# Abolfazlmsl/Oriented-Object-Detection

Hardware: AMD Instinct MI355X
Metric: 416px tiles/sec (whole node), YOLOv11n-OBB 3ch (higher is better)
Workload: dtype f32; 1 GPU; YOLOv11n-OBB 3ch 416x416 tiled inference, single-scale (BASELINE configs[1]): forward + decode + ProbIoU NMS + border filter + per-tile merge + final polygon-IoU merge; step_pipelining=True, nc=12, weights=synthetic seeded, cls bias -8 (no checkpoint offline), final_detections=12170

## Files before the change

### oriented-object-detection_amd/csrc/ctx.h

```cpp
#pragma once
#include <hip/hip_runtime.h>

#include <cstdarg>
#include <cstdint>
#include <cstdio>
#include <map>
#include <memory>
#include <string>
#include <vector>

#include "../../include/obbhip.h"

namespace obb {
struct Model;
struct EngineOpts {
    bool tail = true, tail16 = true, bneck = true, bneck_cv2 = true, c3kimg = true, dwpw = true, upfold = true, stem = true, front = true, pair = true, hmerge = true,
         sppf_fuse = true, attn_mfma = true, xtile = true, nitile = true, nc2 = true, blk32 = true, c3k2f = true, pw32 = true, graph = true;
    int fwd_split = 0 , microbatch = 1024;
};
}

struct obb_ctx {
    int device = 0;
    std::string err;
    struct Slot { void *p = nullptr; size_t bytes = 0; };
    std::vector<Slot> ws;
    std::shared_ptr<obb::Model> model;
    std::map<int, std::shared_ptr<obb::Model>> slots;
    int slot = 0;
    bool opt_f16 = true;
    bool opt_f32 = false;
    obb::EngineOpts opt;
    void *workspace(int slot, size_t bytes);
    ~obb_ctx();
};

namespace obb {
int set_error(obb_ctx *ctx, int code, const char *fmt, ...);
extern thread_local std::string g_tls_error;

#define OBB_HIP(ctx, call)                                                                                  \
    do {                                                                                                    \
        hipError_t e_ = (call);                                                                             \
        if (e_ != hipSuccess)                                                                               \
            return obb::set_error(ctx, OBB_ERR_HIP, "%s failed: %s (%s:%d)", #call, hipGetErrorString(e_), \
                                  __FILE__, __LINE__);                                                      \
    } while (0)

#define OBB_REQUIRE(ctx, cond, ...)                                      \
    do {                                                                 \
        if (!(cond)) return obb::set_error(ctx, OBB_ERR_INVALID, __VA_ARGS__); \
    } while (0)

#define OBB_LAUNCH_CHECK(ctx) OBB_HIP(ctx, hipGetLastError())

enum { WS_GEOM_A = 0, WS_GEOM_B, WS_GEOM_C, WS_GEOM_D, WS_GEOM_E, WS_NMS_A, WS_NMS_B, WS_NMS_C, WS_NMS_D, WS_SURV_A, WS_SURV_B, WS_SEL, WS_DT, WS_TRAIN_A, WS_TRAIN_B, WS_TRAIN_C, WS_TRAIN_D, WS_TRAIN_E, WS_TRAIN_F, WS_COUNT };

inline int64_t cdiv(int64_t a, int64_t b) { return (a + b - 1) / b; }
}
```

### oriented-object-detection_amd/csrc/engine.hip

```cpp
#include <algorithm>
#include <cmath>
#include <cstdlib>
#include <cstring>
#include <map>
#include <memory>
#include <string>
#include <tuple>

#include "bneck.h"
#include "c3k2f32.h"
#include "c3kimg.h"
#include "ctx.h"
#include "dwpw.h"
#include "f32path.h"
#include "front.h"
#include "nnops.h"
#include "pw32.h"
#include "stem.h"

namespace obb {

static constexpr int kRegMax = 16;

struct ConvRecord {
    std::string name;
    int c1, c2, k, s, g, act;
    const float *w, *b;
};

struct Buf {
    int H, W, C;
    bool f32;
    bool virt = false;
    int va_buf = -1, va_co = 0, va_C = 0, vb_buf = -1, vb_co = 0, vb_C = 0;
    int blk = 0;
    int blk32 = 0;
    std::string name;
    int64_t off = 0;
    void *p = nullptr;
    int64_t per_img() const { return (int64_t)H * W * C; }
};

struct Slice { int buf = -1, co = 0, C = 0; };

enum OpType { OP_CONV32, OP_STEM32, OP_C3K2F32, OP_PW32, OP_CONV, OP_DW, OP_POOL, OP_UP, OP_ATTN, OP_STEM, OP_SPPF, OP_BNECK, OP_C3KIMG, OP_DWPW, OP_FRONT };

struct Op {
    OpType type;
    std::string name;
    Slice in, out, res;
    int H = 0, W = 0;
    int Ho = 0, Wo = 0;
    ConvLaunch conv;
    Conv32Launch c32;
    Stem32Launch stem32;
    Pw32Launch pw32;
    C3k2F32Launch c3k2f;
    StemLaunch stem;
    FrontLaunch front;
    BneckLaunch bneck;
    C3kImgLaunch c3kimg;
    DwPwLaunch dwpw;
    double macs = 0;
    bool one_d = false;
    bool vin = false;
    const bf16_t *dw_w = nullptr;
    const float *dw_b = nullptr;
    const float *dw_w32 = nullptr;
    int act = 0;
    int N = 0, nh = 0, kd = 0, hd = 0;
    int head_level = -1;
    bool emit_cmax = false;
    int lane = 0;
    int wait_feat = -1;
    int signal_feat = -1;
};

struct Plan {
    int h = 0, w = 0, A = 0, no = 0, no_pad = 0;
    std::vector<Buf> bufs;
    std::vector<Op> ops;
    std::map<std::string, Slice> named;
    std::vector<void *> dev_allocs;
    int lvl_off[3] = {0, 0, 0};
    int cmax_mask = 0;
    int cap = 0;
    void *slab = nullptr;
    int64_t bytes_per_img = 0;
    double macs_per_img = 0;
    static constexpr int kLanes = 4;
    hipStream_t lanes[kLanes] = {};
    hipEvent_t ev_feat[kLanes] = {}, ev_done[kLanes] = {};
    typedef std::tuple<int, const void *, void *, void *> GraphKey;
    std::map<GraphKey, hipGraphExec_t> graphs;
    std::map<GraphKey, int> seen;
    std::vector<GraphKey> graph_order;
    void drop_graphs() {
        for (auto &kv : graphs) (void)hipGraphExecDestroy(kv.second);
        graphs.clear();
        seen.clear();
        graph_order.clear();
    }
    ~Plan() {
        drop_graphs();
        for (int i = 0; i < kLanes; ++i) {
            if (lanes[i]) (void)hipStreamDestroy(lanes[i]);
            if (ev_feat[i]) (void)hipEventDestroy(ev_feat[i]);
            if (ev_done[i]) (void)hipEventDestroy(ev_done[i]);
        }
        for (void *p : dev_allocs) (void)hipFree(p);
        if (slab) (void)hipFree(slab);
    }
};

struct Model {
// ... 317 lines not shown
            op.name = name + "+" + tail_name;
            P.macs_per_img += (double)op.Ho * op.Wo * r2->c2 * r->c2;
            P.ops.push_back(op);
            if (act16) P.named[tail_name] = out;
            return;
        }
        P.ops.push_back(op);
        P.named[name] = out;
    }

    void dwconv(const std::string &name, Slice in, int H, int W, Slice out, Slice res = Slice()) {
        const ConvRecord *r = rec(name);
        if (!r || err) return;
        if (r->g != r->c1 || r->c1 != r->c2 || r->k != 3 || r->s != 1 || r->c1 != in.C || out.C != in.C) {
            err = set_error(ctx, OBB_ERR_FORMAT, "record %s: not a depthwise 3x3 matching the graph", name.c_str());
            return;
        }
        if (M.f32 && (P.bufs[in.buf].blk32 || P.bufs[out.buf].blk32)) { err = set_error(ctx, OBB_ERR_STATE, "depthwise layer %s on a channel-blocked buffer", name.c_str()); return; }
        int C = in.C;
        std::vector<bf16_t> w((size_t)9 * C + 8, 0);
        std::vector<float> b((size_t)C + 8, 0.f);
        for (int c = 0; c < C; ++c) {
            for (int t = 0; t < 9; ++t) w[(size_t)t * C + c] = host_to_half(r->w[(size_t)c * 9 + t], M.f16);
            b[c] = r->b[c];
        }
        Op op;
        op.type = OP_DW; op.name = name; op.in = in; op.out = out; op.res = res; op.H = H; op.W = W; op.Ho = H; op.Wo = W;
        op.act = r->act;
        if (M.f32) {
            std::vector<float> w32((size_t)9 * C + 8, 0.f);
            for (int c = 0; c < C; ++c)
                for (int t = 0; t < 9; ++t) w32[(size_t)t * C + c] = r->w[(size_t)c * 9 + t];
            op.dw_w32 = upload(w32);
        } else op.dw_w = upload(w);
        op.dw_b = upload(b);
        P.macs_per_img += (double)H * W * C * 9;
        P.ops.push_back(op);
        P.named[name] = out;
    }

    bool dwpw32(const std::string &dwname, const std::string &pwname, Slice in, int H, int W, Slice out, const char *tailname, int head_level) {
        const ConvRecord *rd = rec(dwname), *rp = rec(pwname), *rt = tailname ? rec(tailname) : nullptr;
        if (!(M.tail && M.o.dwpw) || !rd || !rp || (tailname && !rt) || err) return false;
        if (in.buf < 0 || P.bufs[in.buf].virt || rd->g != rd->c1 || rd->c1 != rd->c2 || rd->k != 3 || rd->s != 1 || rd->c1 != in.C || rp->g != 1 || rp->k != 1 || rp->s != 1 ||
            rp->c1 != in.C)
            return false;
        if (rt && (rt->g != 1 || rt->k != 1 || rt->s != 1 || rt->act || rt->c1 != rp->c2 || head_level < 0)) return false;
        if (!rt && (out.buf < 0 || P.bufs[out.buf].virt || out.C != rp->c2)) return false;
        const Conv32Tiling t = plan_dwpw32(in.C, rp->c2, H, W);
        if (t.TH == 0 || (rt && !conv32_tail_supported(t, rp->c2, rt->c2)) || (rt && rt->c2 > 16)) return false;
        Op op;
        op.type = OP_CONV32; op.name = dwname + "+" + pwname + (rt ? std::string("+") + tailname : std::string()); op.in = in; op.out = out;
        op.H = H; op.W = W; op.Ho = H; op.Wo = W; op.head_level = rt ? head_level : -1; op.one_d = false;
        Conv32Launch &L = op.c32;
        L.ks = 1; L.stride = 1; L.cin = in.C; L.cout = rp->c2; L.act = rp->act; L.dw = 1; L.dw_act = rd->act;
        L.TH = t.TH; L.TW = t.TW; L.CK = t.CK; L.WC = t.WC; L.MFM = t.MFM; L.NI = 1;
        L.Hin = L.Hout = H; L.Win = L.Wout = W;
        L.tiles_y = (H + t.TH - 1) / t.TH; L.tiles_x = 1;
        L.wpk = upload(pack_dwpw32_weights(rp->w, rp->c2, in.C, rd->w, rd->b, t));
        std::vector<float> bias32(((size_t)rp->c2 + 63) / 64 * 64 + 64, 0.f);
        for (int c = 0; c < rp->c2; ++c) bias32[c] = rp->b[c];
        L.bias = upload(bias32);
        op.macs = (double)H * W * (9.0 * in.C + (double)in.C * rp->c2);
        if (rt) {
            const Conv32Tiling t2{1, 1, rp->c2, 1, 1, 1};
            L.tail_w = upload(pack_conv32_weights(rt->w, rt->c2, rp->c2, 1, t2, nullptr, false));
            std::vector<float> b2(((size_t)rt->c2 + 63) / 64 * 64 + 64, 0.f);
            for (int c = 0; c < rt->c2; ++c) b2[c] = rt->b[c];
            L.tail_b = upload(b2);
            L.tail_cout = rt->c2; L.tail_act = 0;
            if (out.buf == -2 && out.co == 4 * kRegMax) { op.emit_cmax = true; P.cmax_mask |= 1 << head_level; }
            op.macs += (double)H * W * rt->c1 * rt->c2;
        }
        P.macs_per_img += op.macs;
        P.ops.push_back(op);
        if (!rt) P.named[pwname] = out;
        return true;
    }

    bool dwpw(const std::string &dwname, const std::string &pwname, Slice in, int H, int W, Slice out, const char *tailname = nullptr, int head_level = -1) {
        if (M.f32) return dwpw32(dwname, pwname, in, H, W, out, tailname, head_level);
        const bool on = M.tail && M.o.dwpw;
        const ConvRecord *rd = rec(dwname), *rp = rec(pwname), *rt = tailname ? rec(tailname) : nullptr;
        if (!on || !rd || !rp || (tailname && !rt) || err) return false;
        if (in.buf < 0 || P.bufs[in.buf].blk || P.bufs[in.buf].virt || rd->g != rd->c1 || rd->c1 != rd->c2 || rd->k != 3 || rd->s != 1 || rd->c1 != in.C || !rd->act ||
            rp->g != 1 || rp->k != 1 || rp->s != 1 || !rp->act || rp->c1 != in.C)
            return false;
        if (rt && (rt->g != 1 || rt->k != 1 || rt->s != 1 || rt->act || rt->c1 != rp->c2 || head_level < 0)) return false;
        if (!rt && (out.buf < 0 || P.bufs[out.buf].blk || P.bufs[out.buf].virt || out.C != rp->c2)) return false;
        if (!dwpw_supported(in.C, rp->c2, H, W, rt ? rt->c2 : 0)) return false;
        const int C = in.C;
        Op op;
        op.type = OP_DWPW; op.name = dwname + "+" + pwname + (rt ? std::string("+") + tailname : std::string()); op.in = in; op.out = out;
        op.H = H; op.W = W; op.Ho = H; op.Wo = W; op.head_level = rt ? head_level : -1;
        DwPwLaunch &L = op.dwpw;
        L.H = H; L.W = W; L.cin = C; L.f16 = M.f16;
        std::vector<bf16_t> w((size_t)9 * C + 8, 0);
        std::vector<float> b((size_t)C + 8, 0.f);
        for (int c = 0; c < C; ++c) {
            for (int t = 0; t < 9; ++t) w[(size_t)t * C + c] = host_to_half(rd->w[(size_t)c * 9 + t], M.f16);
            b[c] = rd->b[c];
        }
        L.dw_w = upload(w); L.dw_b = upload(b);
        ConvTiling tp{1, 1, 1, 4, C};
        L.pw_w = upload(pack_conv_weights(rp->w, rp->c2, C, 1, tp, nullptr, 0, M.f16));
        std::vector<float> pb(64 + 64, 0.f);
// ... 462 lines not shown
    }
    *out = it->second.get();
    return OBB_OK;
}

__global__ __launch_bounds__(256) void k_class_max(const float *__restrict__ head, int64_t n, int no_pad, int c0, int nc, float *__restrict__ cmax) {
    const int64_t i = (int64_t)blockIdx.x * 256 + threadIdx.x;
    if (i >= n) return;
    const float *r = head + i * no_pad + c0;
    float m = -INFINITY;
    for (int j = 0; j < nc; ++j) m = fmaxf(m, r[j]);
    cmax[i] = m;
}

static int run_forward(obb_ctx *ctx, Plan &P, const uint8_t *tiles, int B, float *head, float *cmax, hipStream_t st, int boff) {
    Model &M = *ctx->model;
    for (Op &op : P.ops) {
        hipError_t e = hipSuccess;
        switch (op.type) {
            case OP_CONV32: {
                Conv32Launch L = op.c32;
                L.B = B;
                L.xtile = M.o.xtile;
                if (op.in.buf == -1) {
                    L.in.p = (void *)tiles; L.in.bs = (int64_t)P.h * P.w * M.ch; L.in.cs = M.ch; L.in.co = 0;
                } else if (op.vin) {
                    const Buf &vb = P.bufs[op.in.buf];
                    L.in = tref(P, Slice{vb.va_buf, vb.va_co, vb.va_C}, boff);
                    L.in2 = tref(P, Slice{vb.vb_buf, vb.vb_co, vb.vb_C}, boff);
                    L.up_c = vb.va_C; L.up_W = op.W; L.up_HW = op.H * op.W;
                } else L.in = tref(P, op.in, boff);
                TensorRef o;
                int o_hw = 0;
                if (op.head_level >= 0) {
                    o.p = head + (int64_t)P.lvl_off[op.head_level] * P.no_pad;
                    o.bs = (int64_t)P.A * P.no_pad; o.cs = P.no_pad; o.co = op.out.co;
                    if (op.one_d) o_hw = op.Ho * op.Wo;
                } else {
                    o = tref(P, op.out, boff);
                    if (op.one_d && o.cpb) o_hw = op.Ho * op.Wo;
                }
                if (L.tail_cout > 0) { L.tail_out = o; L.tail_out_hw = o_hw; }
                if (cmax && op.emit_cmax) { L.cmax = cmax + P.lvl_off[op.head_level]; L.cmax_bs = P.A; }
                else { L.out = o; L.out_hw = o_hw; }
                L.res = tref(P, op.res, boff);
                if (op.one_d) {
                    const int64_t npx = (int64_t)B * op.Ho * op.Wo;
                    L.B = 1; L.Hin = L.Hout = 1; L.Win = L.Wout = (int)npx;
                    L.tiles_y = 1; L.tiles_x = (int)((npx + L.TW - 1) / L.TW);
                }
                e = launch_conv32(L, st);
                break;
            }
            case OP_PW32: {
                Pw32Launch L = op.pw32;
                L.in = tref(P, op.in, boff); L.out = tref(P, op.out, boff); L.res = tref(P, op.res, boff);
                L.npix = (int64_t)B * op.Ho * op.Wo; L.hw = op.Ho * op.Wo;
                e = launch_pw32(L, st);
                break;
            }
            case OP_C3K2F32: {
                C3k2F32Launch L = op.c3k2f;
                L.B = B; L.cat = tref(P, op.in, boff); L.out = tref(P, op.out, boff);
                e = launch_c3k2f32(L, st);
                break;
            }
            case OP_STEM32: {
                Stem32Launch L = op.stem32;
                L.B = B; L.in = tiles; L.out = tref(P, op.out, boff);
                e = launch_stem32(L, st);
                break;
            }
            case OP_CONV: {
                ConvLaunch L = op.conv;
                L.B = B;
                if (op.in.buf == -1) {
                    L.in.p = (void *)tiles; L.in.bs = (int64_t)P.h * P.w * M.ch; L.in.cs = M.ch; L.in.co = 0;
                } else if (op.vin) {
                    const Buf &vb = P.bufs[op.in.buf];
                    L.in = tref(P, Slice{vb.va_buf, vb.va_co, vb.va_C}, boff);
                    L.in2 = tref(P, Slice{vb.vb_buf, vb.vb_co, vb.vb_C}, boff);
                    L.up_c = vb.va_C; L.up_W = op.W; L.up_HW = op.H * op.W;
                } else L.in = tref(P, op.in, boff);
                if (op.head_level >= 0) {
                    TensorRef hr;
                    hr.p = head + (int64_t)P.lvl_off[op.head_level] * P.no_pad;
                    hr.bs = (int64_t)P.A * P.no_pad; hr.cs = P.no_pad; hr.co = op.out.co;
                    if (L.tail_cout > 0) {
                        L.tail_out = hr;
                        if (op.one_d) L.tail_out_hw = op.Ho * op.Wo;
                    } else {
                        L.out = hr;
                        if (op.one_d) L.out_hw = op.Ho * op.Wo;
                    }
                } else L.out = tref(P, op.out, boff);
                L.res = tref(P, op.res, boff);
                if (op.one_d) {
                    int64_t npx = (int64_t)B * op.Ho * op.Wo;
                    L.B = 1; L.Hin = L.Hout = 1; L.Win = L.Wout = (int)npx;
                    L.tiles_y = 1; L.tiles_x = (int)((npx + L.TW - 1) / L.TW);
                } else if (M.o.nitile) {
                    const int ni = conv_ni_supported(L);
                    if (ni > 1) { L.NI = ni; L.TH = L.Hout; L.TW = L.Wout; L.tiles_x = L.tiles_y = 1; }
                }
                e = launch_conv(L, st);
                break;
// ... 116 lines not shown
extern "C" {

int obb_model_load(obb_ctx *ctx, const void *blob_host, size_t bytes) {
    OBB_REQUIRE(ctx, ctx && blob_host && bytes > 0, "obb_model_load: bad arguments");
    OBB_HIP(ctx, hipSetDevice(ctx->device));
    OBB_HIP(ctx, hipDeviceSynchronize());
    std::shared_ptr<Model> M(new Model());
    M->blob.assign((const char *)blob_host, (const char *)blob_host + bytes);
    int rc = parse_blob(ctx, *M);
    if (rc) return rc;
    M->f16 = ctx->opt_f16;
    M->f32 = ctx->opt_f32;
    M->o = ctx->opt;
    M->tail = ctx->opt.tail;
    M->upfold = ctx->opt.upfold;
    M->hmerge = M->tail && ctx->opt.hmerge;
    M->bneck = M->tail && ctx->opt.bneck;
    if (M->f32) {
        std::vector<float> lut32(256);
        for (int v = 0; v < 256; ++v) lut32[v] = (float)v / 255.0f;
        OBB_HIP(ctx, hipMalloc((void **)&M->lut32_dev, 1024));
        OBB_HIP(ctx, hipMemcpy(M->lut32_dev, lut32.data(), 1024, hipMemcpyHostToDevice));
    }
    std::vector<bf16_t> lut(256);
    for (int v = 0; v < 256; ++v) lut[v] = host_to_half((float)v / 255.0f, M->f16);
    OBB_HIP(ctx, hipMalloc((void **)&M->lut_dev, 512 + 1024));
    OBB_HIP(ctx, hipMemcpy(M->lut_dev, lut.data(), 512, hipMemcpyHostToDevice));
    ctx->model = M;
    return OBB_OK;
}

int obb_model_unload(obb_ctx *ctx, int32_t slot) {
    OBB_REQUIRE(ctx, ctx && slot >= 0 && slot < 64, "obb_model_unload: bad arguments");
    OBB_HIP(ctx, hipSetDevice(ctx->device));
    OBB_HIP(ctx, hipDeviceSynchronize());
    if (slot == ctx->slot) ctx->model.reset();
    ctx->slots.erase(slot);
    return OBB_OK;
}

int obb_set_option(obb_ctx *ctx, const char *key, int64_t value) {
    OBB_REQUIRE(ctx, ctx && key, "obb_set_option: bad arguments");
    std::string k(key);
    if (k == "precision") {
        OBB_REQUIRE(ctx, value == 16 || value == 1016 || value == 32, "obb_set_option: precision must be 16 (fp16), 1016 (bf16) or 32 (fp32)");
        ctx->opt_f16 = (value != 1016);
        ctx->opt_f32 = (value == 32);
        return OBB_OK;
    }
    {
        struct { const char *key; bool *flag; } sw[] = {
            {"tail", &ctx->opt.tail}, {"tail16", &ctx->opt.tail16}, {"bneck", &ctx->opt.bneck}, {"bneck_cv2", &ctx->opt.bneck_cv2},
            {"c3kimg", &ctx->opt.c3kimg}, {"dwpw", &ctx->opt.dwpw}, {"upfold", &ctx->opt.upfold}, {"stem", &ctx->opt.stem}, {"front", &ctx->opt.front}, {"pair", &ctx->opt.pair},
            {"hmerge", &ctx->opt.hmerge}, {"sppf_fuse", &ctx->opt.sppf_fuse}, {"attn_mfma", &ctx->opt.attn_mfma}, {"xtile", &ctx->opt.xtile}, {"nitile", &ctx->opt.nitile}, {"nc2", &ctx->opt.nc2}, {"blk32", &ctx->opt.blk32}, {"c3k2f", &ctx->opt.c3k2f}, {"pw32", &ctx->opt.pw32}, {"graph", &ctx->opt.graph}};
        for (auto &e : sw)
            if (k == e.key) { *e.flag = value != 0; return OBB_OK; }
        if (k == "fuse") return OBB_OK;
        if (k == "fwd_split") { OBB_REQUIRE(ctx, value >= 0 && value <= 4, "obb_set_option: fwd_split must be 0 (auto) .. 4"); ctx->opt.fwd_split = (int)value; return OBB_OK; }
        if (k == "microbatch") { OBB_REQUIRE(ctx, value >= 1 && value <= 1024, "obb_set_option: microbatch must be 1..1024"); ctx->opt.microbatch = (int)value; return OBB_OK; }
    }
    if (k == "model_slot") {
        OBB_REQUIRE(ctx, value >= 0 && value < 64, "obb_set_option: model_slot must be in [0, 64)");
        if ((int)value != ctx->slot) {
            ctx->slots[ctx->slot] = ctx->model;
            ctx->model = ctx->slots[(int)value];
            ctx->slot = (int)value;
        }
        return OBB_OK;
    }
    return set_error(ctx, OBB_ERR_INVALID, "obb_set_option: unknown key '%s'", key);
}

int obb_model_info(const obb_ctx *cctx, int32_t h, int32_t w, int32_t *nc, int32_t *ch, int32_t *anchors, int32_t *nconv) {
    obb_ctx *ctx = const_cast<obb_ctx *>(cctx);
    OBB_REQUIRE(ctx, ctx, "obb_model_info: NULL context");
    if (!ctx->model) return set_error(ctx, OBB_ERR_STATE, "no model loaded");
    if (nc) *nc = ctx->model->nc;
    if (ch) *ch = ctx->model->ch;
    if (nconv) *nconv = (int32_t)ctx->model->nrec_blob;
    if (anchors) {
        OBB_REQUIRE(ctx, h > 0 && w > 0 && h % 32 == 0 && w % 32 == 0, "obb_model_info: h, w must be multiples of 32");
        *anchors = (h / 8) * (w / 8) + (h / 16) * (w / 16) + (h / 32) * (w / 32);
    }
    return OBB_OK;
}

int obb_forward(obb_ctx *ctx, const uint8_t *tiles, int32_t B, int32_t h, int32_t w, float *head, obb_stream_t s) {
    return obb_forward_gate(ctx, tiles, B, h, w, head, nullptr, s);
}

int obb_forward_gate(obb_ctx *ctx, const uint8_t *tiles, int32_t B, int32_t h, int32_t w, float *head, float *cmax, obb_stream_t s) {
    OBB_REQUIRE(ctx, ctx && B >= 0, "obb_forward: bad arguments");
    if (B == 0) return OBB_OK;
    OBB_REQUIRE(ctx, tiles && head, "obb_forward: NULL buffer");
    Plan *P = nullptr;
    int rc = get_plan(ctx, h, w, &P);
    if (rc) return rc;
    const int max_mb = (int)std::min<int64_t>(16384, (int64_t)ctx->opt.microbatch * std::max<int64_t>(1, (416 * 416 + (int64_t)h * w - 1) / ((int64_t)h * w)));
    rc = ensure_capacity(ctx, *P, std::min<int>(B, max_mb));
    if (rc) return rc;
    bool use_graph = ctx->opt.graph;
    {
        hipStreamCaptureStatus cs = hipStreamCaptureStatusNone;
        if (hipStreamIsCapturing((hipStream_t)s, &cs) == hipSuccess && cs != hipStreamCaptureStatusNone) use_graph = false;
    }
    hipStream_t st = (hipStream_t)s;
    const int nrounds = (B + max_mb - 1) / max_mb, per_round = (B + nrounds - 1) / nrounds;
// ... 28 lines not shown
                if (hipGraphInstantiate(&ge, g, nullptr, nullptr, 0) == hipSuccess) {
                    P->graphs[key] = ge;
                    P->graph_order.push_back(key);
                    (void)hipGraphDestroy(g);
                    OBB_HIP(ctx, hipGraphLaunch(ge, st));
                    continue;
                }
                (void)hipGraphDestroy(g);
            }
            (void)hipGetLastError();
            if (rc) return rc;
            rc = run_round(ctx, *P, tp, nb, hp, cp, st);
        }
        if (rc) return rc;
    }
    return OBB_OK;
}

int obb_debug_plan(obb_ctx *ctx, int32_t h, int32_t w, char *buf, int64_t buf_bytes, int64_t *needed) {
    OBB_REQUIRE(ctx, ctx && needed, "obb_debug_plan: bad arguments");
    Plan *P = nullptr;
    int rc = get_plan(ctx, h, w, &P);
    if (rc) return rc;
    std::string out;
    char line[512];
    for (const Op &op : P->ops) {
        double macs = 0;
        const char *ty = "?";
        int grid_x = 0, grid_y = 0, lds = 0;
        switch (op.type) {
            case OP_CONV32: {
                const Conv32Launch &L = op.c32;
                snprintf(line, sizeof line, "conv32 %s k%d s%d cin%d cout%d out%dx%d TH%d TW%d NI%d CK%d WC%d NC%d MFM%d dw%d tail%d vcat%d lds%d macs%.0f\n", op.name.c_str(), L.ks,
                         L.stride, L.cin, L.cout, op.Ho, op.Wo, L.TH, L.TW, L.NI, L.CK, L.WC, L.NC, L.MFM, L.dw, L.tail_cout, op.vin ? 1 : 0, (int)conv32_lds_bytes(L), op.macs);
                break;
            }
            case OP_CONV: {
                ty = "conv";
                const ConvLaunch &L = op.conv;
                macs = (double)op.Ho * op.Wo * L.cout * L.cin * L.ks * L.ks;
                grid_x = op.one_d ? -(op.Ho * op.Wo) : L.tiles_x * L.tiles_y;
                grid_y = (L.cout + 16 * L.NF - 1) / (16 * L.NF);
                lds = (int)conv_lds_bytes(L);
                if (L.tail_cout > 0) macs += (double)op.Ho * op.Wo * L.tail_cout * L.cout;
                const int ni = (!op.one_d && ctx->model->o.nitile) ? conv_ni_supported(L) : 1;
                snprintf(line, sizeof line, "%s %s k%d s%d cin%d cout%d out%dx%d TH%d TW%d MF%d NF%d CK%d NI%d gx%d gy%d lds%d macs%.0f\n", ty,
                         op.name.c_str(), L.ks, L.stride, L.cin, L.cout, op.Ho, op.Wo, ni > 1 ? op.Ho : L.TH, ni > 1 ? op.Wo : L.TW, L.MF, L.NF, L.CK, ni, grid_x, grid_y, lds, macs);
                break;
            }
            case OP_DW: ty = "dwconv"; macs = (double)op.H * op.W * op.in.C * 9;
                snprintf(line, sizeof line, "%s %s c%d out%dx%d macs%.0f\n", ty, op.name.c_str(), op.in.C, op.Ho, op.Wo, macs); break;
            case OP_C3KIMG: snprintf(line, sizeof line, "c3kimg %s c%d out%dx%d macs%.0f\n", op.name.c_str(), op.in.C, op.Ho, op.Wo, op.macs); break;
            case OP_DWPW: snprintf(line, sizeof line, "dwpw %s c%d tail%d out%dx%d macs%.0f\n", op.name.c_str(), op.dwpw.cin, op.dwpw.tail_cout, op.Ho, op.Wo, op.macs); break;
            case OP_BNECK: snprintf(line, sizeof line, "bneck %s c%d co%d out%dx%d rows4 macs%.0f\n", op.name.c_str(), op.bneck.C, op.bneck.CO, op.Ho, op.Wo, op.macs); break;
            case OP_SPPF: snprintf(line, sizeof line, "pool %s c%d out%dx%d x3 macs0\n", op.name.c_str(), op.in.C, op.Ho, op.Wo); break;
            case OP_POOL: snprintf(line, sizeof line, "pool %s c%d out%dx%d macs0\n", op.name.c_str(), op.in.C, op.Ho, op.Wo); break;
            case OP_UP: snprintf(line, sizeof line, "upsample %s c%d out%dx%d macs0\n", op.name.c_str(), op.in.C, op.Ho, op.Wo); break;
            case OP_PW32:
                snprintf(line, sizeof line, "pw32 %s k1 s1 cin%d cout%d out%dx%d waves%d lds%d macs%.0f\n", op.name.c_str(), op.pw32.cin, op.pw32.cout, op.Ho, op.Wo,
                         op.pw32.cin * 256 <= 80 * 1024 ? 8 : 16, op.pw32.cin * 256, op.macs);
                break;
            case OP_C3K2F32: {
                int th, tw;
                c3k2f32_tile(op.H, op.W, th, tw);
                snprintf(line, sizeof line, "c3k2f32 %s c%d co%d out%dx%d TH%d TW%d macs%.0f\n", op.name.c_str(), op.c3k2f.C, op.c3k2f.CO, op.Ho, op.Wo, th, tw, op.macs);
                break;
            }
            case OP_STEM32:
                snprintf(line, sizeof line, "stem32 %s k3 s2 cin%d cout%d out%dx%d rows%d macs%.0f\n", op.name.c_str(), op.stem32.cin, op.stem32.cout, op.Ho, op.Wo, 4, op.macs);
                break;
            case OP_STEM:
                snprintf(line, sizeof line, "stem %s k3 s2 cin%d cout%d out%dx%d rows%d macs%.0f\n", op.name.c_str(), op.stem.cin, op.stem.cout, op.Ho, op.Wo, 4, op.macs);
                break;
            case OP_FRONT: snprintf(line, sizeof line, "front %s cin%d out%dx%d macs%.0f\n", op.name.c_str(), op.front.cin, op.Ho, op.Wo, op.macs); break;
            case OP_ATTN: macs = (double)op.nh * ((double)op.N * op.N * op.kd + (double)op.N * op.N * op.hd);
                snprintf(line, sizeof line, "attn %s N%d nh%d macs%.0f\n", op.name.c_str(), op.N, op.nh, macs); break;
        }
        out += line;
    }
    snprintf(line, sizeof line, "total_macs %.0f bytes_per_img %lld nbufs %zu nops %zu\n", P->macs_per_img, (long long)P->bytes_per_img, P->bufs.size(),
             P->ops.size());
    out += line;
    *needed = (int64_t)out.size() + 1;
    if (buf && buf_bytes >= *needed) memcpy(buf, out.c_str(), out.size() + 1);
    return OBB_OK;
}

int obb_debug_activation(obb_ctx *ctx, int32_t h, int32_t w, int32_t B, const char *name, float *out, int64_t max_elems,
                         int64_t *n_elems, int32_t *shape_hwc_host, obb_stream_t s) {
    OBB_REQUIRE(ctx, ctx && name && n_elems, "obb_debug_activation: bad arguments");
    Plan *P = nullptr;
    int rc = get_plan(ctx, h, w, &P);
    if (rc) return rc;
    auto it = P->named.find(name);
    if (it == P->named.end() || it->second.buf < 0) return set_error(ctx, OBB_ERR_INVALID, "obb_debug_activation: no activation named '%s'", name);
    OBB_REQUIRE(ctx, B <= P->cap, "obb_debug_activation: run obb_forward with B >= %d first", B);
    const Slice &sl = it->second;
    const Buf &b = P->bufs[sl.buf];
    int64_t n = (int64_t)B * b.H * b.W * sl.C;
    *n_elems = n;
    if (shape_hwc_host) { shape_hwc_host[0] = b.H; shape_hwc_host[1] = b.W; shape_hwc_host[2] = sl.C; }
    if (!out) return OBB_OK;
    OBB_REQUIRE(ctx, max_elems >= n, "obb_debug_activation: output too small (%lld < %lld)", (long long)max_elems, (long long)n);
    const int64_t hw = (int64_t)b.H * b.W;
    const int64_t d_bs = b.blk > 0 ? hw * b.blk : b.per_img(), d_ps = b.blk > 0 ? (int64_t)P->cap * hw * b.blk : 0;
    if (b.f32)
// ... 14 lines not shown
```

### oriented-object-detection_amd/ops.py

```python
import ctypes as C
import os
from typing import List, Optional

import torch

from . import _lib

_ctx = {}
T = torch.Tensor


def ctx(device=None):
    idx = torch.cuda.current_device() if device is None else torch.device(device).index or 0
    if idx not in _ctx:
        h = C.c_void_p()
        _lib.check(_lib.lib().obb_ctx_create(idx, C.byref(h)))
        _ctx[idx] = h
    return _ctx[idx]


def destroy_contexts():
    for h in _ctx.values():
        _lib.lib().obb_ctx_destroy(h)
    _ctx.clear()
# ... 509 lines not shown
    return db


def tile_survivors(det, count, lb, tile_ids, rects, margin, iou_thr, strike_cls=1):
    d = _chk(det, torch.float32, "det")
    c = _chk(count, torch.int32, "count")
    ti = _chk(tile_ids, torch.int32, "tile_ids")
    r = _chk(rects, torch.int32, "rects").reshape(-1, 4)
    if lb is not None:
        lb = _chk(lb, torch.float32, "lb").reshape(-1, 3)
    B, md = d.shape[0], d.shape[1]
    rec = torch.empty((B * md, 12), dtype=torch.int32, device=d.device)
    off = torch.empty(B + 1, dtype=torch.int32, device=d.device)
    n = torch.empty(1, dtype=torch.int32, device=d.device)
    _O.tile_survivors(d, c, lb, ti, r, int(margin), int(strike_cls), float(iou_thr), rec, off, n)
    return rec, off, n


def select_kept(order, keep, boxes, cls, conf, angle):
    n = order.shape[0]
    ob = torch.empty((n, 8), dtype=torch.float64, device=order.device)
    oc = torch.empty(n, dtype=torch.int32, device=order.device)
    of = torch.empty(n, dtype=torch.float64, device=order.device)
    oa = torch.empty(n, dtype=torch.float64, device=order.device)
    cnt = torch.empty(1, dtype=torch.int32, device=order.device)
    _O.select_kept(_chk(order, torch.int32, "order"), _chk(keep, torch.uint8, "keep"), _chk(boxes, torch.float64, "boxes"), _chk(cls, torch.int32, "cls"),
                   _chk(conf, torch.float64, "conf"), _chk(angle, torch.float64, "angle"), ob, oc, of, oa, cnt)
    return ob, oc, of, oa, cnt


def records_to_dets(records, n, rects, strike_cls=1):
    rec = _chk(records, torch.int32, "records")
    r = _chk(rects, torch.int32, "rects").reshape(-1, 4)
    n = int(n)
    gb = torch.empty((n, 8), dtype=torch.float64, device=rec.device)
    c = torch.empty(n, dtype=torch.int32, device=rec.device)
    f = torch.empty(n, dtype=torch.float64, device=rec.device)
    a = torch.empty(n, dtype=torch.float64, device=rec.device)
    if n:
        _O.records_to_dets(rec, n, r, int(strike_cls), gb, c, f, a)
    return gb, c, f, a


def gather_compact(recv):
    r = _chk(recv, torch.int32, "recv")
    world, cap = r.shape[0], r.shape[1] - 1
    out = torch.empty((world * cap, 12), dtype=torch.int32, device=r.device)
    counts = torch.empty(world + 1, dtype=torch.int32, device=r.device)
    _O.gather_compact(r, out, counts)
    return out, counts


PRECISIONS = {"f16": 16, "fp16": 16, "bf16": 1016, "f32": 32, "fp32": 32}
MODEL_OPTIONS = ("fuse", "tail", "tail16", "bneck", "bneck_cv2", "c3kimg", "dwpw", "upfold", "stem", "front", "pair", "hmerge", "sppf_fuse", "attn_mfma", "xtile", "nitile", "nc2", "blk32", "c3k2f", "pw32", "graph")


def select_model(slot, device=None):
    _call("obb_set_option", ctx(device), b"model_slot", int(slot))


def model_load(blob, device=None, precision="f16", fuse=False, tail=True, **options):
    c = ctx(device)
    _call("obb_set_option", c, b"precision", PRECISIONS[precision])
    _call("obb_set_option", c, b"fuse", 1 if fuse else 0)
    _call("obb_set_option", c, b"tail", 1 if tail else 0)
    for k in MODEL_OPTIONS[2:]:
        try:
            _call("obb_set_option", c, k.encode(), 1 if options.pop(k, True) else 0)
        except _lib.ObbHipError:
            if not os.environ.get("OBB_LIB"):
                raise
    if options:
        raise TypeError(f"model_load: unknown options {sorted(options)}")
    buf = (C.c_char * len(blob)).from_buffer_copy(blob)
    _call("obb_model_load", c, buf, len(blob))


def model_unload(slot, device=None):
    _call("obb_model_unload", ctx(device), int(slot))


def model_info(h, w, device=None):
    c = ctx(device)
    nc, ch, a, n = C.c_int32(), C.c_int32(), C.c_int32(), C.c_int32()
    _call("obb_model_info", c, h, w, C.byref(nc), C.byref(ch), C.byref(a), C.byref(n))
    return {"nc": nc.value, "ch": ch.value, "anchors": a.value, "nconv": n.value}


def forward(tiles, out=None, cmax=None):
    t = _chk(tiles, torch.uint8, "tiles")
    B, h, w, ch = t.shape
    info = model_info(h, w, t.device)
    if ch != info["ch"]:
        raise ValueError(f"forward: model expects {info['ch']} input channels, got {ch}")
    no = 64 + info["nc"] + 1
    shape = (B, info["anchors"], (no + 3) // 4 * 4)
    if out is not None:
        if tuple(out.shape) != shape:
            raise ValueError(f"forward: out must have shape {shape}")
        head = _chk(out, torch.float32, "out")
    else:
        head = torch.zeros(shape, dtype=torch.float32, device=t.device)
    if cmax is not None:
        cm = _chk(cmax, torch.float32, "cmax")
        if tuple(cm.shape) != shape[:2]:
            raise ValueError(f"forward: cmax must have shape {shape[:2]}")
        if B:
# ... 172 lines not shown
```

Before: 32430 tiles/s.

## Add dedicated f32 depthwise+pointwise fused kernel with MFMA and optional head tail

Adds a new f32 kernel that stages a row tile of input channels in LDS, computes the 3x3 depthwise conv with SiLU on vector ALUs, then feeds the result straight into 16x16x4 f32 MFMAs for the 64-output pointwise conv. It can also apply the detection-head 1x1 tail and a class-max reduction. The engine selects it by default for dw+pw pairs with 64 outputs, replacing the generic conv32 dw path. The aim is less LDS/global traffic and better tile occupancy for these head layers, at the cost of a new code path with fixed tiling, XCD-strided block mapping and extra correctness risk.

```diff
diff --git a/oriented-object-detection_amd/csrc/ctx.h b/oriented-object-detection_amd/csrc/ctx.h
--- a/oriented-object-detection_amd/csrc/ctx.h
+++ b/oriented-object-detection_amd/csrc/ctx.h
@@ -15,7 +15,7 @@
 struct Model;
 struct EngineOpts {
     bool tail = true, tail16 = true, bneck = true, bneck_cv2 = true, c3kimg = true, dwpw = true, upfold = true, stem = true, front = true, pair = true, hmerge = true,
-         sppf_fuse = true, attn_mfma = true, xtile = true, nitile = true, nc2 = true, blk32 = true, c3k2f = true, pw32 = true, graph = true;
+         sppf_fuse = true, attn_mfma = true, xtile = true, nitile = true, nc2 = true, blk32 = true, c3k2f = true, pw32 = true, dwpw32 = true, graph = true;
     int fwd_split = 0 , microbatch = 1024;
 };
 }
diff --git a/oriented-object-detection_amd/csrc/dwpw32.h b/oriented-object-detection_amd/csrc/dwpw32.h
--- /dev/null
+++ b/oriented-object-detection_amd/csrc/dwpw32.h
@@ -0,0 +1,31 @@
+#pragma once
+#include <hip/hip_runtime.h>
+
+#include <vector>
+
+#include "conv.h"
+
+namespace obb {
+
+struct DwPw32Launch {
+    TensorRef in;
+    TensorRef out;
+    const float *pw_w = nullptr;
+    const float *pw_b = nullptr;
+    const float *dw_w = nullptr;
+    int B = 0, H = 0, W = 0, cin = 0, act = 1, dw_act = 1;
+    int TH = 0;
+    const float *tail_w = nullptr;
+    const float *tail_b = nullptr;
+    int tail_cout = 0;
+    TensorRef tail_out;
+    float *cmax = nullptr;
+    int64_t cmax_bs = 0;
+};
+
+int plan_dwpw32s(int cin, int cout, int H, int W);
+std::vector<float> pack_dwpw32s_dw(const float *dw_c9, const float *dw_bias, int cin);
+size_t dwpw32s_lds_bytes(int TH, int W);
+hipError_t launch_dwpw32s(const DwPw32Launch &L, hipStream_t st);
+
+}
diff --git a/oriented-object-detection_amd/csrc/dwpw32.hip b/oriented-object-detection_amd/csrc/dwpw32.hip
--- /dev/null
+++ b/oriented-object-detection_amd/csrc/dwpw32.hip
@@ -0,0 +1,304 @@
+#include "dwpw32.h"
+
+#include <algorithm>
+#include <cmath>
+#include <cstdlib>
+#include <cstring>
+
+namespace obb {
+
+typedef __attribute__((ext_vector_type(4))) float f32x4;
+typedef __attribute__((ext_vector_type(4))) unsigned int u32x4;
+
+struct DwPw32Params {
+    const float *in; int64_t in_bs, in_ps; int in_cs, in_co, in_blk;
+    float *out; int64_t out_bs; int out_cs, out_co;
+    const float *pw_w, *pw_b, *dw_w;
+    const float *w2, *b2; float *out2; int64_t out2_bs; int out2_cs, out2_co, cout2;
+    float *cmax; int64_t cmax_bs;
+    int H, W, cin, nstage, TH, tiles_y, ntiles, per_xcd, act, dw_act;
+    int qs;
+    float inv_blk;
+    int dbg;
+};
+
+#ifdef OBB_DIAG
+#define DW32_DBG(m) (P.dbg & (m))
+#else
+#define DW32_DBG(m) false
+#endif
+
+__device__ __forceinline__ float silu32d(float x) { return x * __builtin_amdgcn_rcpf(1.0f + __expf(-x)); }
+
+static constexpr int kNW = 8, kMF = 2, kSB = 5;
+
+template <int TAIL>
+__global__ __launch_bounds__(kNW * 64, kNW / 2) void k_dwpw_f32(const DwPw32Params P) {
+    extern __shared__ __attribute__((aligned(16))) char smem[];
+    constexpr int NW = kNW, NT = kNW * 64, MF = kMF, SB = kSB;
+    const int tid = threadIdx.x, lane = tid & 63;
+    const int wave = __builtin_amdgcn_readfirstlane(tid >> 6);
+    const int g = lane >> 4, pl = lane & 15;
+    const int xcd = blockIdx.x & 7, lin = blockIdx.x >> 3;
+    const int t = xcd * P.per_xcd + lin;
+    if (lin >= P.per_xcd || t >= P.ntiles) return;
+    const int b = t / P.tiles_y, oy0 = (t - b * P.tiles_y) * P.TH;
+    const int W = P.W, HW = P.H * W;
+    const int npix = min(P.TH, P.H - oy0) * W;
+    const int nfrag = (npix + 15) >> 4;
+    const int in_px = (P.TH + 2) * W;
+    const int nchunk = in_px * 16;
+    const int gp0 = (oy0 - 1) * W;
+
+    int pbase[MF];
+    bool lft[MF], rgt[MF];
+#pragma unroll
+    for (int i = 0; i < MF; ++i) {
+        int p = (wave + NW * i) * 16 + pl;
+        if (p >= npix) p = 0;
+        const int tx = p % W;
+        pbase[i] = p * 16;
+        lft[i] = tx == 0; rgt[i] = tx == W - 1;
+    }
+    if (tid < 32) *reinterpret_cast<float4 *>(smem + (tid & 15) * P.qs + (tid >> 4) * (in_px + 1) * 16) = make_float4(0.f, 0.f, 0.f, 0.f);
+
+    f32x4 acc[4][MF];
+#pragma unroll
+    for (int f = 0; f < 4; ++f)
+#pragma unroll
+        for (int i = 0; i < MF; ++i) acc[f][i] = f32x4{0.f, 0.f, 0.f, 0.f};
+
+    const __amdgpu_buffer_rsrc_t w_rsrc = __builtin_amdgcn_make_buffer_rsrc((void *)P.pw_w, 0, 64 * P.cin * 4, 0x00020000);
+    const __amdgpu_buffer_rsrc_t dw_rsrc = __builtin_amdgcn_make_buffer_rsrc((void *)P.dw_w, 0, 10 * P.cin * 4, 0x00020000);
+    const float *const ib = P.in + (int64_t)b * P.in_bs;
+    const int W16 = W * 16;
+    for (int st = 0; st < P.nstage; ++st) {
+        if (st) __syncthreads();
+        for (int base = 0; base < nchunk; base += NT * SB) {
+            float4 v[SB];
+            int dst[SB];
+#pragma unroll
+            for (int k = 0; k < SB; ++k) {
+                const int idx = base + k * NT + tid;
+                int pix, c;
+                if (P.in_blk) {
+                    const int c8 = (int)(((float)idx + 0.5f) * P.inv_blk), rem = idx - c8 * in_px * 2;
+                    pix = rem >> 1; c = c8 * 2 + (rem & 1);
+                } else { pix = idx >> 4; c = idx & 15; }
+                const int gp = gp0 + pix, ch = st * 64 + c * 4;
+                const bool ok = idx < nchunk && gp >= 0 && gp < HW && !DW32_DBG(1);
+                const float *src = P.in_blk ? ib + (int64_t)(ch >> 3) * P.in_ps + (int64_t)gp * 8 + (ch & 7) : ib + (int64_t)gp * P.in_cs + P.in_co + ch;
+                v[k] = ok ? *reinterpret_cast<const float4 *>(src) : make_float4(0.f, 0.f, 0.f, 0.f);
+                dst[k] = idx < nchunk ? c * P.qs + (1 + pix) * 16 : -1;
+            }
+#pragma unroll
+            for (int k = 0; k < SB; ++k)
+                if (dst[k] >= 0) *reinterpret_cast<float4 *>(smem + dst[k]) = v[k];
+        }
+        __syncthreads();
+
+        const int wso = st * 4096 * 4, dso = st * 64 * 4;
+        auto ldrow = [&](int r, float4 (&dk)[3]) {
+            const int ks = (r * 11) >> 5, ky = r - ks * 3;
+#pragma unroll
+            for (int kx = 0; kx < 3; ++kx) dk[kx] = __builtin_bit_cast(float4, __builtin_amdgcn_raw_buffer_load_b128(dw_rsrc, g * 16, dso + ((ky * 3 + kx) * P.cin + ks * 16) * 4, 0));
+        };
+        float4 dkn[3];
+        ldrow(0, dkn);
+#pragma unroll 1
+        for (int ks = 0; ks < 4; ++ks) {
+            const char *const plane = smem + (ks * 4 + g) * P.qs;
+            float a[MF][4];
+#pragma unroll
+            for (int i = 0; i < MF; ++i) { a[i][0] = 0.f; a[i][1] = 0.f; a[i][2] = 0.f; a[i][3] = 0.f; }
+            f32x4 w[4];
+#pragma unroll 1
+            for (int ky = 0; ky < 3; ++ky) {
+                const float4 dk[3] = {dkn[0], dkn[1], dkn[2]};
+                if (ky == 0) {
+#pragma unroll
+                    for (int f = 0; f < 4; ++f) w[f] = __builtin_bit_cast(f32x4, __builtin_amdgcn_raw_buffer_load_b128(w_rsrc, lane * 16, wso + (f * 1024 + ks * 256) * 4, 0));
+                }
+                ldrow(min(ks * 3 + ky + 1, 11), dkn);
+                if (DW32_DBG(4)) continue;
+#pragma unroll
+                for (int i = 0; i < MF; ++i) {
+                    const int row = pbase[i] + ky * W16;
+                    const float4 v0 = *reinterpret_cast<const float4 *>(plane + (lft[i] ? 0 : row)), v1 = *reinterpret_cast<const float4 *>(plane + row + 16),
+                                 v2 = *reinterpret_cast<const float4 *>(plane + (rgt[i] ? 0 : row + 32));
+                    const float4 vv[3] = {v0, v1, v2};
+#pragma unroll
+                    for (int kx = 0; kx < 3; ++kx) {
+                        a[i][0] = fmaf(vv[kx].x, dk[kx].x, a[i][0]); a[i][1] = fmaf(vv[kx].y, dk[kx].y, a[i][1]);
+                        a[i][2] = fmaf(vv[kx].z, dk[kx].z, a[i][2]); a[i][3] = fmaf(vv[kx].w, dk[kx].w, a[i][3]);
+                    }
+                }
+            }
+            const float4 db = __builtin_bit_cast(float4, __builtin_amdgcn_raw_buffer_load_b128(dw_rsrc, g * 16, dso + (9 * P.cin + ks * 16) * 4, 0));
+            f32x4 d[MF];
+#pragma unroll
+            for (int i = 0; i < MF; ++i) {
+                float o[4] = {a[i][0] + db.x, a[i][1] + db.y, a[i][2] + db.z, a[i][3] + db.w};
+                if (P.dw_act && !DW32_DBG(2)) {
+#pragma unroll
+                    for (int j = 0; j < 4; ++j) o[j] = silu32d(o[j]);
+                }
+                d[i] = f32x4{o[0], o[1], o[2], o[3]};
+            }
+#pragma unroll
+            for (int s = 0; s < 4; ++s)
+#pragma unroll
+                for (int f = 0; f < 4; ++f)
+#pragma unroll
+                    for (int i = 0; i < MF; ++i) {
+                        if (DW32_DBG(8)) { asm volatile("" ::"v"(d[i][s]), "v"(w[f][s])); continue; }
+                        acc[f][i] = __builtin_amdgcn_mfma_f32_16x16x4f32(w[f][s], d[i][s], acc[f][i], 0, 0, 0);
+                    }
+        }
+    }
+
+    const int64_t opix0 = (int64_t)oy0 * W;
+    if constexpr (TAIL == 0) {
+        float4 bv[4];
+#pragma unroll
+        for (int f = 0; f < 4; ++f) bv[f] = *reinterpret_cast<const float4 *>(P.pw_b + f * 16 + g * 4);
+#pragma unroll
+        for (int i = 0; i < MF; ++i) {
+            const int p = (wave + NW * i) * 16 + pl;
+            if (p >= npix) continue;
+            float *op = P.out + (int64_t)b * P.out_bs + (opix0 + p) * P.out_cs + P.out_co + g * 4;
+#pragma unroll
+            for (int f = 0; f < 4; ++f) {
+                float v[4] = {acc[f][i][0] + bv[f].x, acc[f][i][1] + bv[f].y, acc[f][i][2] + bv[f].z, acc[f][i][3] + bv[f].w};
+                if (P.act && !DW32_DBG(2)) {
+#pragma unroll
+                    for (int j = 0; j < 4; ++j) v[j] = silu32d(v[j]);
+                }
+                *reinterpret_cast<float4 *>(op + f * 16) = make_float4(v[0], v[1], v[2], v[3]);
+            }
+        }
+    } else {
+        f32x4 acc2[MF];
+#pragma unroll
+        for (int i = 0; i < MF; ++i) acc2[i] = f32x4{0.f, 0.f, 0.f, 0.f};
+        const float *const w2 = P.w2 + lane * 4;
+#pragma unroll
+        for (int u = 0; u < 4; ++u) {
+            const f32x4 w = *reinterpret_cast<const f32x4 *>(w2 + u * 256);
+            const float4 bv = *reinterpret_cast<const float4 *>(P.pw_b + u * 16 + g * 4);
+            f32x4 av[MF];
+#pragma unroll
+            for (int i = 0; i < MF; ++i) {
+                float v[4] = {acc[u][i][0] + bv.x, acc[u][i][1] + bv.y, acc[u][i][2] + bv.z, acc[u][i][3] + bv.w};
+                if (P.act && !DW32_DBG(2)) {
+#pragma unroll
+                    for (int j = 0; j < 4; ++j) v[j] = silu32d(v[j]);
+                }
+                av[i] = f32x4{v[0], v[1], v[2], v[3]};
+            }
+#pragma unroll
+            for (int s = 0; s < 4; ++s)
+#pragma unroll
+                for (int i = 0; i < MF; ++i)
+                    acc2[i] = __builtin_amdgcn_mfma_f32_16x16x4f32(w[s], av[i][s], acc2[i], 0, 0, 0);
+        }
+        const int c2 = g * 4;
+        const bool lane_on = c2 < P.cout2, full2 = c2 + 4 <= P.cout2;
+        const float4 bv2 = *reinterpret_cast<const float4 *>(P.b2 + (lane_on ? c2 : 0));
+#pragma unroll
+        for (int i = 0; i < MF; ++i) {
+            if (wave + NW * i >= nfrag) continue;
+            const int p = (wave + NW * i) * 16 + pl;
+            const float v[4] = {acc2[i][0] + bv2.x, acc2[i][1] + bv2.y, acc2[i][2] + bv2.z, acc2[i][3] + bv2.w};
+            if (P.cmax) {
+                float m = -INFINITY;
+#pragma unroll
+                for (int j = 0; j < 4; ++j)
+                    if (c2 + j < P.cout2) m = fmaxf(m, v[j]);
+                m = fmaxf(m, __shfl_xor(m, 16));
+                m = fmaxf(m, __shfl_xor(m, 32));
+                if (g == 0 && p < npix) P.cmax[(int64_t)b * P.cmax_bs + opix0 + p] = m;
+            }
+            if (!lane_on || p >= npix) continue;
+            float *op = P.out2 + (int64_t)b * P.out2_bs + (opix0 + p) * P.out2_cs + P.out2_co + c2;
+            if (full2 && ((P.out2_cs | P.out2_co) & 3) == 0) {
+                *reinterpret_cast<float4 *>(op) = make_float4(v[0], v[1], v[2], v[3]);
+            } else {
+#pragma unroll
+                for (int j = 0; j < 4; ++j)
+                    if (c2 + j < P.cout2) op[j] = v[j];
+            }
+        }
+    }
+}
+
+static int npx_planes(int TH, int W) { return ((TH + 2) * W + 2) | 1; }
+size_t dwpw32s_lds_bytes(int TH, int W) { return (size_t)npx_planes(TH, W) * 256; }
+
+int plan_dwpw32s(int cin, int cout, int H, int W) {
+    if (cin < 64 || cin % 64 || cout != 64 || H < 1 || W < 2 || W > 256) return 0;
+    int best = 0;
+    int64_t best_cost = -1;
+    for (int th = 1; th <= std::min(H, 16 * kNW * kMF / W); ++th) {
+        if (dwpw32s_lds_bytes(th, W) > 80 * 1024) break;
+        const int64_t cost = (int64_t)((H + th - 1) / th) * (((th * W + 15) / 16 + kNW - 1) / kNW);
+        if (best_cost < 0 || cost <= best_cost) { best_cost = cost; best = th; }
+    }
+    return best;
+}
+
+std::vector<float> pack_dwpw32s_dw(const float *dw_c9, const float *dw_bias, int cin) {
+    std::vector<float> out((size_t)10 * cin + 64, 0.f);
+    for (int c = 0; c < cin; ++c) {
+        for (int tp = 0; tp < 9; ++tp) out[(size_t)tp * cin + c] = dw_c9[(size_t)c * 9 + tp];
+        out[(size_t)9 * cin + c] = dw_bias[c];
+    }
+    return out;
+}
+
+hipError_t launch_dwpw32s(const DwPw32Launch &L, hipStream_t st) {
+    if (L.B < 1 || L.H < 1 || L.W < 2 || L.cin < 64 || L.cin % 64 || L.TH < 1 || L.TH > L.H || L.TH * L.W > 16 * kNW * kMF) return hipErrorInvalidValue;
+    if (!L.in.p || !L.pw_w || !L.pw_b || !L.dw_w) return hipErrorInvalidValue;
+    const size_t lds = dwpw32s_lds_bytes(L.TH, L.W);
+    if (lds > 80 * 1024) return hipErrorInvalidValue;
+    DwPw32Params P;
+    memset(&P, 0, sizeof P);
+    P.in = (const float *)L.in.p; P.in_bs = L.in.bs; P.in_cs = L.in.cs; P.in_co = L.in.co;
+    if (L.in.cpb) {
+        if (L.in.cpb != 2 || L.in.cs != 8 || L.in.co % 8 || L.in.ps <= 0) return hipErrorInvalidValue;
+        P.in_blk = 1; P.in_ps = L.in.ps; P.in += (int64_t)(L.in.co >> 3) * L.in.ps; P.in_co = 0;
+    } else if ((L.in.cs & 3) || (L.in.co & 3)) return hipErrorInvalidValue;
+    P.pw_w = L.pw_w; P.pw_b = L.pw_b; P.dw_w = L.dw_w;
+    P.H = L.H; P.W = L.W; P.cin = L.cin; P.nstage = L.cin / 64; P.TH = L.TH; P.act = L.act; P.dw_act = L.dw_act;
+    P.tiles_y = (L.H + L.TH - 1) / L.TH;
+    const int64_t ntiles = (int64_t)L.B * P.tiles_y;
+    if (ntiles + 8 >= (1ll << 28)) return hipErrorInvalidValue;
+    P.ntiles = (int)ntiles; P.per_xcd = (int)((ntiles + 7) / 8);
+    P.qs = npx_planes(L.TH, L.W) * 16;
+    P.inv_blk = 1.0f / (float)((L.TH + 2) * L.W * 2);
+    if (L.tail_cout > 0) {
+        if (L.tail_cout > 16 || !L.tail_w || !L.tail_b || !L.tail_out.p || L.tail_out.cpb || L.out.p) return hipErrorInvalidValue;
+        P.w2 = L.tail_w; P.b2 = L.tail_b; P.cout2 = L.tail_cout;
+        P.out2 = (float *)L.tail_out.p; P.out2_bs = L.tail_out.bs; P.out2_cs = L.tail_out.cs; P.out2_co = L.tail_out.co;
+        P.cmax = L.cmax; P.cmax_bs = L.cmax_bs;
+    } else {
+        if (!L.out.p || L.out.cpb || (L.out.cs & 3) || (L.out.co & 3) || L.cmax) return hipErrorInvalidValue;
+        P.out = (float *)L.out.p; P.out_bs = L.out.bs; P.out_cs = L.out.cs; P.out_co = L.out.co;
+    }
+    static bool attr_set[2] = {false, false};
+    const int ti = L.tail_cout > 0 ? 1 : 0;
+    if (!attr_set[ti]) {
+        const hipError_t e = hipFuncSetAttribute(ti ? (const void *)k_dwpw_f32<1> : (const void *)k_dwpw_f32<0>, hipFuncAttributeMaxDynamicSharedMemorySize, 80 * 1024);
+        if (e != hipSuccess) return e;
+        attr_set[ti] = true;
+    }
+#ifdef OBB_DIAG
+    { static const int dbg = getenv("OBB_DW32_DBG") ? atoi(getenv("OBB_DW32_DBG")) : 0; P.dbg = dbg; }
+#endif
+    const dim3 grid((unsigned)(P.per_xcd * 8));
+    if (ti) hipLaunchKernelGGL((k_dwpw_f32<1>), grid, dim3(kNW * 64), lds, st, P);
+    else hipLaunchKernelGGL((k_dwpw_f32<0>), grid, dim3(kNW * 64), lds, st, P);
+    return hipGetLastError();
+}
+
+}
diff --git a/oriented-object-detection_amd/csrc/engine.hip b/oriented-object-detection_amd/csrc/engine.hip
--- a/oriented-object-detection_amd/csrc/engine.hip
+++ b/oriented-object-detection_amd/csrc/engine.hip
@@ -12,6 +12,7 @@
 #include "c3kimg.h"
 #include "ctx.h"
 #include "dwpw.h"
+#include "dwpw32.h"
 #include "f32path.h"
 #include "front.h"
 #include "nnops.h"
@@ -43,7 +44,7 @@
 
 struct Slice { int buf = -1, co = 0, C = 0; };
 
-enum OpType { OP_CONV32, OP_STEM32, OP_C3K2F32, OP_PW32, OP_CONV, OP_DW, OP_POOL, OP_UP, OP_ATTN, OP_STEM, OP_SPPF, OP_BNECK, OP_C3KIMG, OP_DWPW, OP_FRONT };
+enum OpType { OP_CONV32, OP_STEM32, OP_C3K2F32, OP_PW32, OP_CONV, OP_DW, OP_POOL, OP_UP, OP_ATTN, OP_STEM, OP_SPPF, OP_BNECK, OP_C3KIMG, OP_DWPW, OP_FRONT, OP_DWPW32 };
 
 struct Op {
     OpType type;
@@ -61,6 +62,7 @@
     BneckLaunch bneck;
     C3kImgLaunch c3kimg;
     DwPwLaunch dwpw;
+    DwPw32Launch dwpw32s;
     double macs = 0;
     bool one_d = false;
     bool vin = false;
@@ -484,6 +486,33 @@
         Op op;
         op.type = OP_CONV32; op.name = dwname + "+" + pwname + (rt ? std::string("+") + tailname : std::string()); op.in = in; op.out = out;
         op.H = H; op.W = W; op.Ho = H; op.Wo = W; op.head_level = rt ? head_level : -1; op.one_d = false;
+        const int th32 = (M.o.dwpw32 && (!rt || out.buf == -2)) ? plan_dwpw32s(in.C, rp->c2, H, W) : 0;
+        if (th32 > 0) {
+            op.type = OP_DWPW32;
+            DwPw32Launch &D = op.dwpw32s;
+            D.H = H; D.W = W; D.cin = in.C; D.act = rp->act; D.dw_act = rd->act; D.TH = th32;
+            const Conv32Tiling tp{1, 1, 64, 4, 1, 1, 1};
+            D.pw_w = upload(pack_conv32_weights(rp->w, rp->c2, in.C, 1, tp, nullptr, false));
+            std::vector<float> pb(64 + 64, 0.f);
+            for (int c = 0; c < rp->c2; ++c) pb[c] = rp->b[c];
+            D.pw_b = upload(pb);
+            D.dw_w = upload(pack_dwpw32s_dw(rd->w, rd->b, in.C));
+            op.macs = (double)H * W * (9.0 * in.C + (double)in.C * rp->c2);
+            if (rt) {
+                const Conv32Tiling t2{1, 1, rp->c2, 1, 1, 1};
+                D.tail_w = upload(pack_conv32_weights(rt->w, rt->c2, rp->c2, 1, t2, nullptr, false));
+                std::vector<float> b2(((size_t)rt->c2 + 63) / 64 * 64 + 64, 0.f);
+                for (int c = 0; c < rt->c2; ++c) b2[c] = rt->b[c];
+                D.tail_b = upload(b2);
+                D.tail_cout = rt->c2;
+                if (out.co == 4 * kRegMax) { op.emit_cmax = true; P.cmax_mask |= 1 << head_level; }
+                op.macs += (double)H * W * rt->c1 * rt->c2;
+            }
+            P.macs_per_img += op.macs;
+            P.ops.push_back(op);
+            if (!rt) P.named[pwname] = out;
+            return true;
+        }
         Conv32Launch &L = op.c32;
         L.ks = 1; L.stride = 1; L.cin = in.C; L.cout = rp->c2; L.act = rp->act; L.dw = 1; L.dw_act = rd->act;
         L.TH = t.TH; L.TW = t.TW; L.CK = t.CK; L.WC = t.WC; L.MFM = t.MFM; L.NI = 1;
@@ -1052,6 +1081,20 @@
                 e = launch_conv32(L, st);
                 break;
             }
+            case OP_DWPW32: {
+                DwPw32Launch L = op.dwpw32s;
+                L.B = B;
+                L.in = tref(P, op.in, boff);
+                if (L.tail_cout > 0) {
+                    TensorRef o;
+                    o.p = head + (int64_t)P.lvl_off[op.head_level] * P.no_pad;
+                    o.bs = (int64_t)P.A * P.no_pad; o.cs = P.no_pad; o.co = op.out.co;
+                    L.tail_out = o;
+                    if (cmax && op.emit_cmax) { L.cmax = cmax + P.lvl_off[op.head_level]; L.cmax_bs = P.A; }
+                } else L.out = tref(P, op.out, boff);
+                e = launch_dwpw32s(L, st);
+                break;
+            }
             case OP_PW32: {
                 Pw32Launch L = op.pw32;
                 L.in = tref(P, op.in, boff); L.out = tref(P, op.out, boff); L.res = tref(P, op.res, boff);
@@ -1274,7 +1317,7 @@
         struct { const char *key; bool *flag; } sw[] = {
             {"tail", &ctx->opt.tail}, {"tail16", &ctx->opt.tail16}, {"bneck", &ctx->opt.bneck}, {"bneck_cv2", &ctx->opt.bneck_cv2},
             {"c3kimg", &ctx->opt.c3kimg}, {"dwpw", &ctx->opt.dwpw}, {"upfold", &ctx->opt.upfold}, {"stem", &ctx->opt.stem}, {"front", &ctx->opt.front}, {"pair", &ctx->opt.pair},
-            {"hmerge", &ctx->opt.hmerge}, {"sppf_fuse", &ctx->opt.sppf_fuse}, {"attn_mfma", &ctx->opt.attn_mfma}, {"xtile", &ctx->opt.xtile}, {"nitile", &ctx->opt.nitile}, {"nc2", &ctx->opt.nc2}, {"blk32", &ctx->opt.blk32}, {"c3k2f", &ctx->opt.c3k2f}, {"pw32", &ctx->opt.pw32}, {"graph", &ctx->opt.graph}};
+            {"hmerge", &ctx->opt.hmerge}, {"sppf_fuse", &ctx->opt.sppf_fuse}, {"attn_mfma", &ctx->opt.attn_mfma}, {"xtile", &ctx->opt.xtile}, {"nitile", &ctx->opt.nitile}, {"nc2", &ctx->opt.nc2}, {"blk32", &ctx->opt.blk32}, {"c3k2f", &ctx->opt.c3k2f}, {"pw32", &ctx->opt.pw32}, {"dwpw32", &ctx->opt.dwpw32}, {"graph", &ctx->opt.graph}};
         for (auto &e : sw)
             if (k == e.key) { *e.flag = value != 0; return OBB_OK; }
         if (k == "fuse") return OBB_OK;
@@ -1409,6 +1452,10 @@
                 snprintf(line, sizeof line, "%s %s c%d out%dx%d macs%.0f\n", ty, op.name.c_str(), op.in.C, op.Ho, op.Wo, macs); break;
             case OP_C3KIMG: snprintf(line, sizeof line, "c3kimg %s c%d out%dx%d macs%.0f\n", op.name.c_str(), op.in.C, op.Ho, op.Wo, op.macs); break;
             case OP_DWPW: snprintf(line, sizeof line, "dwpw %s c%d tail%d out%dx%d macs%.0f\n", op.name.c_str(), op.dwpw.cin, op.dwpw.tail_cout, op.Ho, op.Wo, op.macs); break;
+            case OP_DWPW32:
+                snprintf(line, sizeof line, "dwpw32 %s cin%d cout64 tail%d out%dx%d TH%d lds%d macs%.0f\n", op.name.c_str(), op.dwpw32s.cin, op.dwpw32s.tail_cout, op.Ho, op.Wo,
+                         op.dwpw32s.TH, (int)dwpw32s_lds_bytes(op.dwpw32s.TH, op.W), op.macs);
+                break;
             case OP_BNECK: snprintf(line, sizeof line, "bneck %s c%d co%d out%dx%d rows4 macs%.0f\n", op.name.c_str(), op.bneck.C, op.bneck.CO, op.Ho, op.Wo, op.macs); break;
             case OP_SPPF: snprintf(line, sizeof line, "pool %s c%d out%dx%d x3 macs0\n", op.name.c_str(), op.in.C, op.Ho, op.Wo); break;
             case OP_POOL: snprintf(line, sizeof line, "pool %s c%d out%dx%d macs0\n", op.name.c_str(), op.in.C, op.Ho, op.Wo); break;
diff --git a/oriented-object-detection_amd/ops.py b/oriented-object-detection_amd/ops.py
--- a/oriented-object-detection_amd/ops.py
+++ b/oriented-object-detection_amd/ops.py
@@ -585,7 +585,7 @@
 
 
 PRECISIONS = {"f16": 16, "fp16": 16, "bf16": 1016, "f32": 32, "fp32": 32}
-MODEL_OPTIONS = ("fuse", "tail", "tail16", "bneck", "bneck_cv2", "c3kimg", "dwpw", "upfold", "stem", "front", "pair", "hmerge", "sppf_fuse", "attn_mfma", "xtile", "nitile", "nc2", "blk32", "c3k2f", "pw32", "graph")
+MODEL_OPTIONS = ("fuse", "tail", "tail16", "bneck", "bneck_cv2", "c3kimg", "dwpw", "upfold", "stem", "front", "pair", "hmerge", "sppf_fuse", "attn_mfma", "xtile", "nitile", "nc2", "blk32", "c3k2f", "pw32", "dwpw32", "graph")
 
 
 def select_model(slot, device=None):
```

Result: no change. 32480 tiles/s (median of 6 runs) (+0.1%).
